# MrTornado24/FENeRF

Hardware: AMD Instinct MI355X
Metric: rays/s/GPU forward render (128x128, 24+24 samples, H=256 FiLM-SIREN + 32x96^3 grid) (higher is better)
Workload: dtype f16x3 (error-compensated fp16 MFMA, fp32 accumulate; fp32-class accuracy); 1 GPU; configs[1]: CelebA_double_semantic_texture_embedding_256_dim_96 generator, 128x128, 24+24 hierarchical samples, batch 1/GPU, forward-only render, procedural weights; img_size=128, num_steps=24, batch_per_gpu=1

## Files before the change

fenerf_amd/csrc/fenerf_siren_f16w.hip:

```cpp
#include <hip/hip_runtime.h>

#include <type_traits>

#include "fenerf_composite_ray.h"
#include "fenerf_film.h"
#include "fenerf_internal.h"
#include "fenerf_launch.h"
#include "fenerf_layout.h"
#include "fenerf_trig.h"
#include "fenerf_wave16.h"

namespace fenerf {
namespace w16 {

using namespace wave16;

typedef _Float16 half8 __attribute__((ext_vector_type(8)));
typedef _Float16 half4 __attribute__((ext_vector_type(4)));
typedef _Float16 half2 __attribute__((ext_vector_type(2)));

#define MFMA16W(a, b, c) __builtin_amdgcn_mfma_f32_16x16x32_f16((a), (b), (c), 0, 0, 0)

__device__ __forceinline__ half8 as_half8(const float4& v) { return __builtin_bit_cast(half8, v); }
template <int MODE> struct TapeW { const char* base; };
struct TapeQ { unsigned q[4]; };
__device__ __forceinline__ unsigned phase_u16(float theta) {
  const float v = __builtin_amdgcn_fractf(theta) * 65536.f;
  const unsigned c = __builtin_bit_cast(unsigned, v + 8388608.f) & 0xffffu;
  return !(__builtin_fabsf(theta) < __builtin_inff()) ? TAPE16_NONFINITE : (c == TAPE16_NONFINITE ? (v < 65535.f ? 0xfffeu : 0u) : c);
}
#ifndef FENERF_EXP_DEPHASE
#define FENERF_EXP_DEPHASE 0
#endif

struct WStream {
  bool skip;
  unsigned long long g_next;
  unsigned voff;
  unsigned ring_lds;
  const char* ring_lane;
  bool early;
};

__device__ __forceinline__ void ws_issue(WStream& w, int slot) {
  const unsigned m0 = w.ring_lds + (unsigned)slot * (CH * 1024);
  if (!w.skip) glds_1k_s(reinterpret_cast<const void*>(w.g_next), w.voff, m0);
  w.g_next += CH * 1024;
}

template <bool LO = true>
__device__ __forceinline__ AK ws_read(const WStream& w, int slot, int spl) {
  AK a;
  if (LO) ring_read_lo(a, w.ring_lane, slot, spl);
  else { a.lo[0] = make_float4(0.f, 0.f, 0.f, 0.f); a.lo[1] = a.lo[0]; }
  ring_read_hi(a, w.ring_lane, slot, spl);
  return a;
}

__device__ __forceinline__ void ws_step(WStream& w, int i, bool early) {
  const bool sync = (i & 1) == 0;
  if (sync) {
    wait_vmcnt<DPF - 3>();
    __builtin_amdgcn_s_barrier();
  }
  LDS_FENCE();
  if (early)
    ws_issue(w, (i + DPF) % NSLOT);
}
__device__ __forceinline__ void ws_issue_late(WStream& w, int i, bool early) {
  if (!early) ws_issue(w, (i + DPF) % NSLOT);
}

template <bool LO = true>
__device__ __forceinline__ void kstep_mfma(f32x4 (&acc)[2], const AK& a, const half8& bh, const half8& bl) {
  if (LO) {
    acc[0] = MFMA16W(as_half8(a.lo[0]), bh, acc[0]);
    acc[1] = MFMA16W(as_half8(a.lo[1]), bh, acc[1]);
  }
  acc[0] = MFMA16W(as_half8(a.hi[0]), bl, acc[0]);
  acc[1] = MFMA16W(as_half8(a.hi[1]), bl, acc[1]);
  acc[0] = MFMA16W(as_half8(a.hi[0]), bh, acc[0]);
  acc[1] = MFMA16W(as_half8(a.hi[1]), bh, acc[1]);
}

struct FilmQ { float2 f, p; };
template <int PF4>
__device__ __forceinline__ FilmQ epi_load(int nbp, int piece, const float* film) {
  const int rt = piece >> 1, pc = piece & 1;
  FilmQ q;
  q.f = *reinterpret_cast<const float2*>(film + 32 * nbp + 8 * rt + 2 * pc);
  q.p = *reinterpret_cast<const float2*>(film + PF4 + 32 * nbp + 8 * rt + 2 * pc);
  return q;
}
template <int KS, int SAVE>
__device__ __forceinline__ void epi_compute(const f32x4 (&acc)[2], int nbp, int piece, const FilmQ& q, half8 (&yh)[KS],
                                            half8 (&yl)[KS], TapeW<SAVE> tw, int tile_odd, TapeQ& tq) {
  const int rt = piece >> 1, pc = piece & 1;
  const float2 f = q.f, p = q.p;
  if (SAVE == 1 && pc == 0) {
    const int lo = opaque((int)(threadIdx.x & 63));
    const unsigned toff = (unsigned)(((2 * (lo >> 5)) * 64 + ((lo >> 4) & 1) * 32 + 16 * tile_odd + (lo & 15)) * 16);
    st_f4_nt(tw.base + (nbp * 4 + rt) * 1024, toff, acc[rt]);
  }
  const float th0 = __builtin_fmaf(f.x, acc[rt][2 * pc + 0], p.x), th1 = __builtin_fmaf(f.y, acc[rt][2 * pc + 1], p.y);
  if (SAVE == 2) {
    tq.q[piece] = __builtin_amdgcn_perm(phase_u16(th1), phase_u16(th0), 0x05040100u);
    if (piece == 3) {
      const int lo = opaque((int)(threadIdx.x & 63));
      const u32x4 v = {tq.q[0], tq.q[1], tq.q[2], tq.q[3]};
      st_u4_nt(tw.base + nbp * 2048, (unsigned)(1024 * tile_odd + 16 * lo), v);
    }
  }
  const float s0 = sin2pi(th0);
  const float s1 = sin2pi(th1);
  const _Float16 h0 = (_Float16)__builtin_fmaf(s0, F16_ACT_SCALE, 0.f), h1 = (_Float16)__builtin_fmaf(s1, F16_ACT_SCALE, 0.f);
  half2 hp = {h0, h1}, lp = {(_Float16)__builtin_fmaf(s0, F16_ACT_SCALE, -(float)h0), (_Float16)__builtin_fmaf(s1, F16_ACT_SCALE, -(float)h1)};
  asm volatile("" : "+v"(hp), "+v"(lp));
  const int s = 4 * rt + 2 * pc;
  yh[nbp][s] = hp[0]; yh[nbp][s + 1] = hp[1];
  yl[nbp][s] = lp[0]; yl[nbp][s + 1] = lp[1];
}
template <int KS, int PF4, int SAVE>
__device__ __forceinline__ void epi_piece(const f32x4 (&acc)[2], int nbp, int piece, const float* film, half8 (&yh)[KS],
                                          half8 (&yl)[KS], TapeW<SAVE> tw, int tile_odd, TapeQ& tq) {
  epi_compute<KS, SAVE>(acc, nbp, piece, epi_load<PF4>(nbp, piece, film), yh, yl, tw, tile_odd, tq);
}
template <int KS, int PF4, int SAVE>
__device__ __forceinline__ void epi_all(const f32x4 (&acc)[2], int nbp, const float* film, half8 (&yh)[KS], half8 (&yl)[KS],
                                        TapeW<SAVE> tw, int tile_odd) {
  TapeQ tq;
#pragma unroll
  for (int pc = 0; pc < 4; ++pc) epi_piece<KS, PF4, SAVE>(acc, nbp, pc, film, yh, yl, tw, tile_odd, tq);
}

struct APipe { AK c, n; };
struct FilmQ2 { FilmQ q[4]; };
template <bool LOR = true, bool LOM = true, int PH = -1, class BOP, class LOADQ, class PIECE>
__device__ __forceinline__ void chunk_step(f32x4 (&acc)[2], APipe& a, WStream& ws, int i, int sp0, BOP bop, LOADQ loadq, PIECE piece) {
  const bool early = PH < 0 ? ws.early : PH == 0;
  constexpr int PSPL = (PH == 1 && FENERF_EXP_DEPHASE == 1) ? 0 : 1;
  ws_step(ws, i, early);
  FilmQ2 fq;
#pragma unroll
  for (int spl = 0; spl < 2; ++spl) {
    if (spl == 1) ws_issue_late(ws, i, early);
    if (spl == 0) loadq(fq);
    const AK nn = ws_read<LOR>(ws, (i + 1) % NSLOT, spl);
    __builtin_amdgcn_sched_barrier(0);
    half8 bh, bl;
    if (bop(sp0 + spl, bh, bl)) kstep_mfma<LOR && LOM>(acc, a.c, bh, bl);
    if (spl == PSPL) piece(fq);
    a.c = a.n;
    a.n = nn;
    __builtin_amdgcn_sched_barrier(0);
  }
}
template <bool LO = true, int PH = -1>
__device__ __forceinline__ void chunk_skip(APipe& a, WStream& ws, int i) {
  const bool early = PH < 0 ? ws.early : PH == 0;
  ws_step(ws, i, early);
  ws_issue_late(ws, i, early);
  a.c = ws_read<LO>(ws, (i + 1) % NSLOT, 0);
  a.n = ws_read<LO>(ws, (i + 1) % NSLOT, 1);
  __builtin_amdgcn_sched_barrier(0);
}

template <int QB>
__device__ __forceinline__ void piece_range(int qc, int& p0, int& p1) {
  constexpr int QBE = QB < 4 ? QB : 4;
  if (qc >= QBE) { p0 = p1 = 0; return; }
  p0 = 4 * qc / QBE;
  p1 = 4 * (qc + 1) / QBE;
}

template <bool FUSED> struct FuseArgs {};
template <> struct FuseArgs<true> {
  int rays_per_group, octs_per_group;
  long long groups, total_rays;
  float* z_fine;
  float* out_fine;
  CompositeParams coarse;
  CompositeParams final_;
};
#ifndef FENERF_EXP_RAY_PHASE
#define FENERF_EXP_RAY_PHASE 2
#endif
#ifndef FENERF_EXP_FUSED_MAXM
#define FENERF_EXP_FUSED_MAXM 128
#endif
constexpr int FUSED_MAXM = FENERF_EXP_FUSED_MAXM;

template <int H, bool GRID, int SAVE, bool FUSED = false, int TERMS2 = 0>
__global__ __launch_bounds__(512, 2) void siren16w_kernel(SirenParams P, int n_geo, int n_color, int n_lab, int C, FuseArgs<FUSED> F) {
  static_assert(!(FUSED && SAVE != 0), "the fused render is the no-grad path");
  static_assert(TERMS2 == 0 || (SAVE == 0 && !FUSED), "the reduced-precision forwards are plain no-grad evaluations");
  constexpr bool LOR = TERMS2 != 1;
  constexpr bool LOC = TERMS2 == 0;
  constexpr int NB = H / 32, KS = H / 32;
  constexpr int QB = (KS + 1) / 2;
  constexpr int C0_KS = KS + (GRID ? 1 : 0) + 1;
  constexpr int C0_QB = (2 * (2 * KS + (GRID ? 2 : 0) + 1) + CH - 1) / CH;
  constexpr int SQ_CHUNKS = pad_stage(NB * QB * CH) / CH;
  constexpr int C0_CHUNKS = pad_stage(NB * C0_QB * CH) / CH;
  constexpr int HEAD_CHUNKS = pad_stage(QB * CH) / CH;
  extern __shared__ __attribute__((aligned(16))) float4 smem[];

  if (P.clk && threadIdx.x == 0) {
    P.clk[(size_t)blockIdx.x * 4 + 0] = __builtin_amdgcn_s_memtime();
    P.clk[(size_t)blockIdx.x * 4 + 1] = __builtin_amdgcn_s_memrealtime();
  }
  const int lane = threadIdx.x & 63;
  const int wave = __builtin_amdgcn_readfirstlane(threadIdx.x >> 6);
  const int n = lane & 15, g = lane >> 4;
  const int L = n_geo + n_color;
  const int stage_f4 = (16 * C + 3) / 4;
  char* lds = reinterpret_cast<char*>(smem);
  char* ring = lds;
  constexpr int FILM_F = H * 4 < 1024 ? 1024 : H * 4;
  constexpr int FILM_BYTES = 2 * FILM_F;
  char* film_base = lds + NSLOT * CH * 1024 + wave * (2 * FILM_BYTES);
  float* l0_lds = reinterpret_cast<float*>(lds + NSLOT * CH * 1024 + NWAVE * 2 * FILM_BYTES);
  float* cst = l0_lds + NB * 256;
  float* stage = cst + 80 + wave * stage_f4 * 4;
  float4* ext_wave = reinterpret_cast<float4*>(cst + 80 + NWAVE * stage_f4 * 4) + wave * 256;

  for (int i = threadIdx.x; i < NB * 256; i += 512) l0_lds[i] = P.stream[i];
  if (threadIdx.x < 32) {
    cst[threadIdx.x] = P.consts[CONST_FILM_BIAS + (size_t)2 * L * H + threadIdx.x];
    cst[32 + threadIdx.x] = P.consts[CONST_HEAD_BIAS + threadIdx.x];
  } else if (threadIdx.x < 36) {
    cst[64 + threadIdx.x - 32] = P.consts[CONST_FILM_BIAS + (size_t)2 * L * H + threadIdx.x];
    cst[68 + threadIdx.x - 32] = P.consts[CONST_RGB_BIAS + threadIdx.x - 32];
  }
  CompositeParams* ray_par = reinterpret_cast<CompositeParams*>(reinterpret_cast<float4*>(cst + 80 + NWAVE * stage_f4 * 4) + NWAVE * 256);
  if constexpr (FUSED) {
    constexpr int NW = (int)(sizeof(CompositeParams) / 4);
    static_assert(sizeof(CompositeParams) % 4 == 0 && NW <= 256, "copied one dword per thread");
    const int t = threadIdx.x & 255;
    const unsigned* src = reinterpret_cast<const unsigned*>(threadIdx.x < 256 ? &F.coarse : &F.final_);
    if (t < NW) reinterpret_cast<unsigned*>(ray_par + (threadIdx.x >> 8))[t] = src[t];
  }
  wait_vmcnt<0>();
  __syncthreads();

  WStream ws;
  {
    const int spl = wave >> 2, rt = (wave >> 1) & 1, hl = wave & 1;
    const int gi = n >> 2, r = n & 3;
    const int row = 16 * (gi >> 1) + 4 * (gi & 1) + 8 * rt + r;
    const int e_old = 2 * (2 * spl + (g >> 1)) + hl;
    ws.voff = e_old * 1024 + ((g & 1) * 32 + row) * 16;
  }
  const unsigned long long g_stream = reinterpret_cast<unsigned long long>(P.stream + P.ring_offset_floats);
  ws.g_next = g_stream;
  ws.ring_lds = __builtin_amdgcn_readfirstlane(lds_addr(ring) + wave * 1024);
  ws.ring_lane = ring + lane * 16;
  ws.early = wave < NWAVE / 2;
  ws.skip = TERMS2 == 1 && (wave & 1);

  const long long ntiles = (P.P + 15) / 16;
  const long long nocts = (ntiles + NWAVE - 1) / NWAVE;
  int opg = 1;
  long long nunits = nocts;
  if constexpr (FUSED) { opg = F.octs_per_group; nunits = F.groups; }
  const int nblk = gridDim.x;
  const int nx = nblk < 8 ? nblk : 8;
  const int xcd = blockIdx.x % nx, bi = blockIdx.x / nx;
  const int blocks_in_x = nblk / nx + (xcd < nblk % nx ? 1 : 0);
  const long long o_begin = nunits * xcd / nx, o_end = nunits * (xcd + 1) / nx;

  if (P.raw_fg && o_begin + bi < o_end) {
    const long long p_first = (o_begin + bi) * opg * (NWAVE * 16);
    long long p_last = o_end * opg * (NWAVE * 16) - 1;
    if (p_last >= P.P) p_last = P.P - 1;
    film_prep_prologue(P, p_first / P.pts_per_image, p_last / P.pts_per_image, H, n_geo, n_color);
  }

#pragma unroll
  for (int i = 0; i < DPF; ++i) ws_issue(ws, i);
  wait_vmcnt<DPF - 1>();
  __builtin_amdgcn_s_barrier();
  LDS_FENCE();
  if (wave >= NWAVE / 2) __builtin_amdgcn_s_setprio(1);
  APipe a_cur;
  a_cur.c = ws_read<LOR>(ws, 0, 0);
  a_cur.n = ws_read<LOR>(ws, 0, 1);

  for (long long unit = o_begin + bi; unit < o_end; unit += blocks_in_x) {
  const int nsub = FUSED ? 2 * opg : 1;
#pragma unroll 1
  for (int sub = 0; sub < nsub; ++sub) {
    const bool fine_pass = FUSED && sub >= opg;
    const long long oct = FUSED ? unit * opg + (fine_pass ? sub - opg : sub) : unit;
    const float* z_src = P.z;
    float* out_dst = P.out;
    if constexpr (FUSED) {
      if (fine_pass) { z_src = F.z_fine; out_dst = F.out_fine; }
    }
    ws.g_next = g_stream + (unsigned long long)DPF * (CH * 1024);
    const long long tile = oct * NWAVE + wave;
    long long pt = tile * 16 + n;
    if (pt >= P.P) pt = P.P - 1;
    const long long img = __builtin_amdgcn_readfirstlane((int)(pt / P.pts_per_image));
    float px, py, pz, dx, dy, dz;
    if (P.points) {
      px = P.points[pt * 3 + 0]; py = P.points[pt * 3 + 1]; pz = P.points[pt * 3 + 2];
      if (P.pdirs) { dx = P.pdirs[pt * 3 + 0]; dy = P.pdirs[pt * 3 + 1]; dz = P.pdirs[pt * 3 + 2]; }
      else { dx = 0.f; dy = 0.f; dz = -1.f; }
    } else {
      const long long ray = pt / P.n_per_ray;
      const float zz = z_src[pt];
      const float ox = P.origins[ray * 3 + 0], oy = P.origins[ray * 3 + 1], oz = P.origins[ray * 3 + 2];
      dx = P.dirs[ray * 3 + 0]; dy = P.dirs[ray * 3 + 1]; dz = P.dirs[ray * 3 + 2];
      px = __fadd_rn(ox, __fmul_rn(dx, zz)); py = __fadd_rn(oy, __fmul_rn(dy, zz)); pz = __fadd_rn(oz, __fmul_rn(dz, zz));
      if (P.lock_view) { dx = 0.f; dy = 0.f; dz = -1.f; }
    }
    const float qx = px * P.box_scale, qy = py * P.box_scale, qz = pz * P.box_scale;
    constexpr int TL = SAVE == 2 ? H * 64 : H * 128;
    const int tile_odd = (int)(tile & 1);
    const char* tape_tile = SAVE ? uniform_ptr(reinterpret_cast<const char*>(P.tape) + (size_t)(tile >> 1) * L * TL) : nullptr;
    auto tape_of = [&](int layer) {
      TapeW<SAVE> t{SAVE ? uniform_ptr(tape_tile + (size_t)layer * TL) : nullptr};
      if (SAVE) asm volatile("s_nop 4" ::: "memory");
      return t;
    };

    const float* fp_img = P.fp + (size_t)img * L * H;
    const float* pp_img = P.pp + (size_t)img * L * H;
    auto film_issue = [&](int layer) {
      const unsigned dst = __builtin_amdgcn_readfirstlane(lds_addr(film_base) + (layer & 1) * FILM_BYTES);
      const float* gf = fp_img + (size_t)layer * H;
      const float* gp = pp_img + (size_t)layer * H;
      const unsigned vo = (unsigned)opaque(lane) * 16;
      for (int off = 0; off < H * 4; off += 1024) {
        glds_1k_s(reinterpret_cast<const char*>(gf) + off, vo, dst + off);
        glds_1k_s(reinterpret_cast<const char*>(gp) + off, vo, dst + FILM_F + off);
      }
    };
    film_issue(0);
    if (L > 1) film_issue(1);

    float e[8];
#pragma unroll
    for (int i = 0; i < 8; ++i) e[i] = 0.f;
    if (GRID) {
      const int ch0 = 16 * (g & 1) + 8 * (g >> 1);
      const float ix = ((qx + 1.f) / 2.f) * (float)(P.gw - 1);
      const float iy = ((qy + 1.f) / 2.f) * (float)(P.gh - 1);
      const float iz = ((qz + 1.f) / 2.f) * (float)(P.gd - 1);
      const float x0 = floorf(ix), y0 = floorf(iy), z0 = floorf(iz);
#pragma unroll
      for (int c = 0; c < 8; ++c) {
        const int cz = c >> 2, cy = (c >> 1) & 1, cx = c & 1;
        const float xi = x0 + cx, yi = y0 + cy, zi = z0 + cz;
        const float wx = cx ? (ix - x0) : (x0 + 1.f - ix);
        const float wy = cy ? (iy - y0) : (y0 + 1.f - iy);
        const float wz = cz ? (iz - z0) : (z0 + 1.f - iz);
        const float wgt = wx * wy * wz;
        const bool ok = xi >= 0.f && xi <= (float)(P.gw - 1) && yi >= 0.f && yi <= (float)(P.gh - 1) && zi >= 0.f &&
                        zi <= (float)(P.gd - 1);
        if (ok) {
          const long long vox = ((long long)(int)zi * P.gh + (int)yi) * P.gw + (int)xi;
          const float4* gp = reinterpret_cast<const float4*>(P.grid + vox * 32 + ch0);
#pragma unroll
          for (int q = 0; q < 2; ++q) {
            const float4 v = gp[q];
            e[4 * q + 0] += v.x * wgt; e[4 * q + 1] += v.y * wgt; e[4 * q + 2] += v.z * wgt; e[4 * q + 3] += v.w * wgt;
          }
        }
      }
    }
    if (SAVE && GRID) {
      float4* ep = reinterpret_cast<float4*>(P.tape_e + pt * 32 + 16 * (g & 1) + 8 * (g >> 1));
      ep[0] = make_float4(e[0], e[1], e[2], e[3]);
      ep[1] = make_float4(e[4], e[5], e[6], e[7]);
    }
    {
      half8 eh, el, dh, dl;
#pragma unroll
      for (int t = 0; t < 8; ++t) {
        const float v = e[t] * F16_ACT_SCALE;
        const _Float16 hh = (_Float16)v;
        eh[t] = hh; el[t] = (_Float16)(v - (float)hh);
      }
      const float d3[3] = {dx * F16_ACT_SCALE, dy * F16_ACT_SCALE, dz * F16_ACT_SCALE};
#pragma unroll
      for (int t = 0; t < 8; ++t) { dh[t] = (_Float16)0.f; dl[t] = (_Float16)0.f; }
#pragma unroll
      for (int t = 0; t < 3; ++t) {
        const float v = g == 0 ? d3[t] : 0.f;
        const _Float16 hh = (_Float16)v;
        dh[t] = hh; dl[t] = (_Float16)(v - (float)hh);
      }
      float4* ext = ext_wave + lane;
      ext[0] = __builtin_bit_cast(float4, eh); ext[64] = __builtin_bit_cast(float4, el);
      ext[128] = __builtin_bit_cast(float4, dh); ext[192] = __builtin_bit_cast(float4, dl);
    }
    wait_vmcnt<0>();
    LDS_FENCE();

    auto film_lane = [&](int layer) -> const float* {
      const int gq = opaque(lane) >> 4;
      return reinterpret_cast<const float*>(film_base + (layer & 1) * FILM_BYTES) + 16 * (gq >> 1) + 4 * (gq & 1);
    };

    half8 xh[KS], xl[KS];
    {
      const float b = g == 0 ? qx : (g == 1 ? qy : (g == 2 ? qz : 0.f));
      const int gi = n >> 2, r = n & 3;
      const float* wl = l0_lds + ((g & 1) * 32 + 16 * (gi >> 1) + 4 * (gi & 1) + r) * 4 + (g >> 1);
      const TapeW<SAVE> tw0 = tape_of(0);
#pragma unroll
      for (int nb = 0; nb < NB; ++nb) {
        f32x4 acc[2];
#pragma unroll
        for (int rt = 0; rt < 2; ++rt) {
          const f32x4 z4 = {0.f, 0.f, 0.f, 0.f};
          acc[rt] = MFMA32W(wl[nb * 256 + 8 * rt * 4], b, z4);
        }
        epi_all<KS, FILM_F / 4, SAVE>(acc, nb, film_lane(0), xh, xl, tw0, tile_odd);
      }
    }
    auto film_layer = [&](auto ph_c, int l) {
      constexpr int PH = decltype(ph_c)::value;
      const float* ff = film_lane(l);
      const TapeW<SAVE> tw = tape_of(l);
      half8 yh[KS], yl[KS];
      if (l + 1 < L) film_issue(l + 1);
      if (SQ_CHUNKS < DPF + 2) wait_vmcnt<0>();
      if (l == n_geo) {
        const float4* ext = ext_wave + opaque(lane);
        auto bop0 = [&](int sp, half8& bh, half8& bl) -> bool {
          if (sp < KS) { bh = xh[sp]; bl = xl[sp]; return true; }
          if (GRID && sp == KS) { bh = as_half8(ext[0]); bl = as_half8(ext[64]); return true; }
          if (sp == C0_KS - 1) { bh = as_half8(ext[128]); bl = as_half8(ext[192]); return true; }
          return false;
        };
        f32x4 acc_prev[2] = {{0.f, 0.f, 0.f, 0.f}, {0.f, 0.f, 0.f, 0.f}};
        TapeQ tq;
#pragma unroll
        for (int nb = 0; nb < NB; ++nb) {
          f32x4 acc[2] = {{0.f, 0.f, 0.f, 0.f}, {0.f, 0.f, 0.f, 0.f}};
#pragma unroll
          for (int qc = 0; qc < C0_QB; ++qc) {
            chunk_step<LOR, LOC, PH>(acc, a_cur, ws, nb * C0_QB + qc, 2 * qc, bop0, [&](FilmQ2& fq) {
              if (nb > 0) {
                int p0, p1;
                piece_range<C0_QB>(qc, p0, p1);
#pragma unroll
                for (int pc = 0; pc < 4; ++pc)
                  if (pc >= p0 && pc < p1) fq.q[pc] = epi_load<FILM_F / 4>(nb - 1, pc, ff);
              }
            }, [&](const FilmQ2& fq) {
              if (nb > 0) {
                int p0, p1;
                piece_range<C0_QB>(qc, p0, p1);
#pragma unroll
                for (int pc = 0; pc < 4; ++pc)
                  if (pc >= p0 && pc < p1) epi_compute<KS, SAVE>(acc_prev, nb - 1, pc, fq.q[pc], yh, yl, tw, tile_odd, tq);
              }
            });
          }
          acc_prev[0] = acc[0]; acc_prev[1] = acc[1];
        }
#pragma unroll
        for (int i = NB * C0_QB; i < C0_CHUNKS; ++i) chunk_skip<LOR, PH>(a_cur, ws, i);
        epi_all<KS, FILM_F / 4, SAVE>(acc_prev, NB - 1, ff, yh, yl, tw, tile_odd);
        {
          f32x4 acc[2] = {{0.f, 0.f, 0.f, 0.f}, {0.f, 0.f, 0.f, 0.f}};
          auto bop = [&](int sp, half8& bh, half8& bl) -> bool {
            if (sp < KS) { bh = xh[sp]; bl = xl[sp]; return true; }
            return false;
          };
#pragma unroll
          for (int qc = 0; qc < QB; ++qc) chunk_step<LOR, true, PH>(acc, a_cur, ws, qc, 2 * qc, bop, [](FilmQ2&) {}, [](const FilmQ2&) {});
#pragma unroll
          for (int i = QB; i < HEAD_CHUNKS; ++i) chunk_skip<LOR, PH>(a_cur, ws, i);
          const int lane_o = opaque(lane);
          const int n_o = lane_o & 15, f_o = 16 * (lane_o >> 5) + 4 * ((lane_o >> 4) & 1);
#pragma unroll
          for (int rt = 0; rt < 2; ++rt) {
#pragma unroll
            for (int r = 0; r < 4; ++r) {
              const int row = f_o + 8 * rt + r;
              if (row <= n_lab) {
                const int ch = row < n_lab ? row : C - 1;
                stage[n_o * C + ch] = acc[rt][r] * cst[row] + cst[32 + row];
              }
            }
          }
        }
      } else {
        auto square_stage = [&](auto lom_c) {
        constexpr bool LOM = decltype(lom_c)::value;
        auto bop = [&](int sp, half8& bh, half8& bl) -> bool {
          if (sp < KS) { bh = xh[sp]; bl = xl[sp]; return true; }
          return false;
        };
        f32x4 acc_prev[2] = {{0.f, 0.f, 0.f, 0.f}, {0.f, 0.f, 0.f, 0.f}};
        TapeQ tq;
#pragma unroll
        for (int nb = 0; nb < NB; ++nb) {
          f32x4 acc[2] = {{0.f, 0.f, 0.f, 0.f}, {0.f, 0.f, 0.f, 0.f}};
#pragma unroll
          for (int qc = 0; qc < QB; ++qc) {
            chunk_step<LOR, LOM, PH>(acc, a_cur, ws, nb * QB + qc, 2 * qc, bop, [&](FilmQ2& fq) {
              if (nb > 0) {
                int p0, p1;
                piece_range<QB>(qc, p0, p1);
#pragma unroll
                for (int pc = 0; pc < 4; ++pc)
                  if (pc >= p0 && pc < p1) fq.q[pc] = epi_load<FILM_F / 4>(nb - 1, pc, ff);
              }
            }, [&](const FilmQ2& fq) {
              if (nb > 0) {
                int p0, p1;
                piece_range<QB>(qc, p0, p1);
#pragma unroll
                for (int pc = 0; pc < 4; ++pc)
                  if (pc >= p0 && pc < p1) epi_compute<KS, SAVE>(acc_prev, nb - 1, pc, fq.q[pc], yh, yl, tw, tile_odd, tq);
              }
            });
          }
          acc_prev[0] = acc[0]; acc_prev[1] = acc[1];
        }
#pragma unroll
        for (int i = NB * QB; i < SQ_CHUNKS; ++i) chunk_skip<LOR, PH>(a_cur, ws, i);
        epi_all<KS, FILM_F / 4, SAVE>(acc_prev, NB - 1, ff, yh, yl, tw, tile_odd);
        };
        if constexpr (TERMS2 == 2) {
          if (l < n_geo) square_stage(std::true_type{}); else square_stage(std::false_type{});
        } else {
          square_stage(std::integral_constant<bool, LOR>{});
        }
      }
#pragma unroll
      for (int k = 0; k < KS; ++k) { xh[k] = yh[k]; xl[k] = yl[k]; }
    };
#pragma unroll 1
    for (int l = 1; l < L; ++l) {
#if FENERF_WAVE_HALF_COPIES
      if (ws.early) film_layer(std::integral_constant<int, 0>{}, l); else film_layer(std::integral_constant<int, 1>{}, l);
#else
      film_layer(std::integral_constant<int, -1>{}, l);
#endif
    }
    {
      constexpr int PH = -1;
      f32x4 acc[2] = {{0.f, 0.f, 0.f, 0.f}, {0.f, 0.f, 0.f, 0.f}};
      auto bop = [&](int sp, half8& bh, half8& bl) -> bool {
        if (sp < KS) { bh = xh[sp]; bl = xl[sp]; return true; }
        return false;
      };
#pragma unroll
      for (int qc = 0; qc < QB; ++qc) chunk_step<LOR, LOC, PH>(acc, a_cur, ws, qc, 2 * qc, bop, [](FilmQ2&) {}, [](const FilmQ2&) {});
#pragma unroll
      for (int i = QB; i < HEAD_CHUNKS; ++i) chunk_skip<LOR, PH>(a_cur, ws, i);
      const int lane_o = opaque(lane);
      const int n_o = lane_o & 15;
      if ((lane_o >> 4) == 0) {
#pragma unroll
        for (int r = 0; r < 3; ++r) {
          const float v = acc[0][r] * cst[64 + r] + cst[68 + r];
          stage[n_o * C + (C - 4) + r] = 1.f / (1.f + __expf(-v));
        }
      }
    }
    __builtin_amdgcn_fence(__ATOMIC_RELEASE, "wavefront");
    __builtin_amdgcn_wave_barrier();
    __builtin_amdgcn_fence(__ATOMIC_ACQUIRE, "wavefront");
    {
      const long long base = tile * 16 * C;
      const long long limit = P.P * C;
      for (int i = opaque(lane); i < 16 * C; i += 64)
        if (base + i < limit) out_dst[base + i] = stage[i];
    }
    wait_vmcnt<0>();
    __builtin_amdgcn_wave_barrier();
    if constexpr (FUSED) {
      if (FENERF_EXP_RAY_PHASE > 0 && (sub == opg - 1 || sub == nsub - 1)) {
        __builtin_amdgcn_fence(__ATOMIC_RELEASE, "workgroup");
        __builtin_amdgcn_s_barrier();
        __builtin_amdgcn_fence(__ATOMIC_ACQUIRE, "workgroup");
        float* sc = reinterpret_cast<float*>(ext_wave);
        float* s_z = sc;
        float* s_zs = sc + FUSED_MAXM;
        int* s_ord = reinterpret_cast<int*>(sc + 2 * FUSED_MAXM + 4);
        float* s_w = sc + 3 * FUSED_MAXM + 4;
        const int lane_r = opaque(lane);
        const long long ray0 = unit * F.rays_per_group;
        for (int r = wave; r < F.rays_per_group; r += NWAVE) {
          const long long ray = ray0 + r;
          if (FENERF_EXP_RAY_PHASE > 1 && ray < F.total_rays) {
#pragma unroll 1
            for (int rep = 0; rep < (FENERF_EXP_RAY_PHASE > 2 ? 2 : 1); ++rep) {
              if (!fine_pass) composite_ray<false, FUSED_MAXM>(ray_par[0], ray, lane_r, s_z, s_zs, s_ord, s_w);
              else composite_ray<true, FUSED_MAXM>(ray_par[1], ray, lane_r, s_z, s_zs, s_ord, s_w);
              __builtin_amdgcn_wave_barrier();
            }
          }
          __builtin_amdgcn_wave_barrier();
        }
        if (!fine_pass) {
          __builtin_amdgcn_fence(__ATOMIC_RELEASE, "workgroup");
          __builtin_amdgcn_s_barrier();
          __builtin_amdgcn_fence(__ATOMIC_ACQUIRE, "workgroup");
        }
        wait_vmcnt<0>();
      }
    }
  }
  }
  wait_vmcnt<0>();
  __builtin_amdgcn_s_barrier();
  if (P.clk && threadIdx.x == 0) {
    P.clk[(size_t)blockIdx.x * 4 + 2] = __builtin_amdgcn_s_memtime();
    P.clk[(size_t)blockIdx.x * 4 + 3] = __builtin_amdgcn_s_memrealtime();
  }
}

static size_t lds_bytes_16w(const FenerfModel* m, int H) {
  const int stage_f4 = (16 * m->C + 3) / 4;
  const size_t film_f = H * 4 < 1024 ? 1024 : H * 4;
  return (size_t)NSLOT * CH * 1024 + (size_t)NWAVE * 2 * (2 * film_f) + (size_t)(H / 32) * 1024 + 80 * 4 +
         (size_t)NWAVE * stage_f4 * 16 + (size_t)NWAVE * 4096;
}

template <int H, bool GRID>
static int launch_fused_t(const FenerfModel* m, const SirenParams& p, const FuseArgs<true>& F, int blocks, void* stream) {
  const size_t lds = lds_bytes_16w(m, H) + (2 * sizeof(CompositeParams) + 255) / 256 * 256;
  auto kfn = siren16w_kernel<H, GRID, 0, true>;
  if (int rc = ensure_dynamic_lds(reinterpret_cast<const void*>(kfn), lds)) return rc;
  hipLaunchKernelGGL(kfn, dim3((unsigned)blocks), dim3(512), lds, (hipStream_t)stream, p, m->n_geo, m->n_color, m->n_lab, m->C, F);
  return check_launch("fused render launch");
}

template <int H, bool GRID, int SAVE, int TERMS2 = 0>
static int launch_t(const FenerfModel* m, const SirenParams& p, void* stream) {
  const size_t lds = lds_bytes_16w(m, H);
  auto kfn = siren16w_kernel<H, GRID, SAVE, false, TERMS2>;
  if (int rc = ensure_dynamic_lds(reinterpret_cast<const void*>(kfn), lds)) return rc;
  const unsigned blocks = persistent_blocks((p.P + 15) / 16, NWAVE, m->num_cus);
  hipLaunchKernelGGL(kfn, dim3(blocks), dim3(512), lds, (hipStream_t)stream, p, m->n_geo, m->n_color, m->n_lab, m->C, FuseArgs<false>{});
  return check_launch("siren16w launch");
}

}

static int launch_siren16w_one(const FenerfModel* m, const SirenParams& q, void* stream) {
  return dispatch_width(m->H, m->grid_ch != 0, [&](auto h, auto g) {
    constexpr int H = decltype(h)::value;
    constexpr bool GRID = decltype(g)::value;
    if (q.tape && q.tape_format == FENERF_TAPE_U16) return w16::launch_t<H, GRID, 2>(m, q, stream);
    if (q.tape) return w16::launch_t<H, GRID, 1>(m, q, stream);
    if (m->forward_mode == FENERF_FORWARD_F16X2) return w16::launch_t<H, GRID, 0, 1>(m, q, stream);
    if (m->forward_mode == FENERF_FORWARD_F16X3_COLOR_X2) return w16::launch_t<H, GRID, 0, 2>(m, q, stream);
    return w16::launch_t<H, GRID, 0>(m, q, stream);
  });
}

bool fused_render_plan(const FenerfModel* m, long long B, long long R, int N, bool balanced_only, FusedRenderPlan* plan) {
  if (m->precision != FENERF_PREC_F16X3 || N < 3 || 2 * N > w16::FUSED_MAXM) return false;
  if (m->forward_mode != FENERF_FORWARD_F16X3) return false;
  int g = N, b = 128;
  while (b) { const int t = g % b; g = b; b = t; }
  const int G = 128 / g, opg = N / g;
  if (R % G != 0) return false;
  const long long groups = B * R / G, nocts = groups * opg;
  const long long cus = launch_cus(m);
  const long long blocks_f = groups < cus ? groups : cus, blocks_p = nocts < cus ? nocts : cus;
  if (balanced_only && (groups + blocks_f - 1) / blocks_f * opg > (nocts + blocks_p - 1) / blocks_p) return false;
  plan->rays_per_group = G; plan->octs_per_group = opg; plan->groups = groups; plan->blocks = (int)blocks_f;
  return true;
}

int launch_render16w_fused(const FenerfModel* m, const SirenParams& p, const FusedRenderPlan& plan, float* z_fine, float* out_fine,
                           const CompositeParams& coarse, const CompositeParams& final_, void* stream) {
  w16::FuseArgs<true> F;
  F.rays_per_group = plan.rays_per_group; F.octs_per_group = plan.octs_per_group; F.groups = plan.groups;
  F.total_rays = coarse.BR;
  F.z_fine = z_fine; F.out_fine = out_fine; F.coarse = coarse; F.final_ = final_;
  return dispatch_width(m->H, m->grid_ch != 0, [&](auto h, auto g) {
    return w16::launch_fused_t<decltype(h)::value, decltype(g)::value>(m, p, F, plan.blocks, stream);
  });
}

int launch_siren16w(const FenerfModel* m, const SirenParams& p, void* stream) {
  if (p.P <= 0) return FENERF_OK;
  if (p.pts_per_image % 32 == 0 || p.P == p.pts_per_image) return launch_siren16w_one(m, p, stream);
  const long long nimg = p.P / p.pts_per_image;
  const int L = m->L, H = m->H;
  for (long long b = 0; b < nimg; ++b) {
    SirenParams q = p;
    q.P = p.pts_per_image;
    q.fp = p.fp + (size_t)b * L * H;
    q.pp = p.pp + (size_t)b * L * H;
    if (p.raw_fg) {
      q.raw_fg = p.raw_fg + (size_t)b * m->n_geo * H; q.raw_pg = p.raw_pg + (size_t)b * m->n_geo * H;
      q.raw_fa = p.raw_fa + (size_t)b * m->n_color * H; q.raw_pa = p.raw_pa + (size_t)b * m->n_color * H;
      q.n_images = 1;
    }
    q.out = p.out + (size_t)b * p.pts_per_image * m->C;
    if (p.points) {
      q.points = p.points + (size_t)b * p.pts_per_image * 3;
      if (p.pdirs) q.pdirs = p.pdirs + (size_t)b * p.pts_per_image * 3;
    } else {
      const long long rays = p.pts_per_image / p.n_per_ray;
      q.origins = p.origins + (size_t)b * rays * 3;
      q.dirs = p.dirs + (size_t)b * rays * 3;
      q.z = p.z + (size_t)b * p.pts_per_image;
    }
    int rc = launch_siren16w_one(m, q, stream);
    if (rc) return rc;
  }
  return FENERF_OK;
}

}
```

Before: 6.055 million rays/s.

## Carry last output block's epilogue into next layer's MFMA chunks

Defers the sine/FiLM epilogue of each layer's final output block (nb=NB-1) and interleaves it with the first MFMA chunks of the next layer, so the tail epilogue no longer sits serialized after the matmul. The next layer's first chunks only consume the earlier K-slices, which are already finalized. FiLM prefetch for layer l+1 is moved later to match, epi_all now batches its loads before a scheduling barrier, and the trailing vmcnt wait is restricted to the fused path. This adds register pressure from the carried accumulators and tape state, plus ordering complexity around the K-slice dependency.

```diff
diff --git a/fenerf_amd/csrc/fenerf_siren_f16w.hip b/fenerf_amd/csrc/fenerf_siren_f16w.hip
--- a/fenerf_amd/csrc/fenerf_siren_f16w.hip
+++ b/fenerf_amd/csrc/fenerf_siren_f16w.hip
@@ -121,16 +121,15 @@
   yl[nbp][s] = lp[0]; yl[nbp][s + 1] = lp[1];
 }
 template <int KS, int PF4, int SAVE>
-__device__ __forceinline__ void epi_piece(const f32x4 (&acc)[2], int nbp, int piece, const float* film, half8 (&yh)[KS],
-                                          half8 (&yl)[KS], TapeW<SAVE> tw, int tile_odd, TapeQ& tq) {
-  epi_compute<KS, SAVE>(acc, nbp, piece, epi_load<PF4>(nbp, piece, film), yh, yl, tw, tile_odd, tq);
-}
-template <int KS, int PF4, int SAVE>
 __device__ __forceinline__ void epi_all(const f32x4 (&acc)[2], int nbp, const float* film, half8 (&yh)[KS], half8 (&yl)[KS],
                                         TapeW<SAVE> tw, int tile_odd) {
   TapeQ tq;
-#pragma unroll
-  for (int pc = 0; pc < 4; ++pc) epi_piece<KS, PF4, SAVE>(acc, nbp, pc, film, yh, yl, tw, tile_odd, tq);
+  FilmQ q[4];
+#pragma unroll
+  for (int pc = 0; pc < 4; ++pc) q[pc] = epi_load<PF4>(nbp, pc, film);
+  __builtin_amdgcn_sched_barrier(0);
+#pragma unroll
+  for (int pc = 0; pc < 4; ++pc) epi_compute<KS, SAVE>(acc, nbp, pc, q[pc], yh, yl, tw, tile_odd, tq);
 }
 
 struct APipe { AK c, n; };
@@ -203,6 +202,7 @@
   constexpr int SQ_CHUNKS = pad_stage(NB * QB * CH) / CH;
   constexpr int C0_CHUNKS = pad_stage(NB * C0_QB * CH) / CH;
   constexpr int HEAD_CHUNKS = pad_stage(QB * CH) / CH;
+  constexpr bool CARRY = QB >= 2;
   extern __shared__ __attribute__((aligned(16))) float4 smem[];
 
   if (P.clk && threadIdx.x == 0) {
@@ -405,6 +405,25 @@
     };
 
     half8 xh[KS], xl[KS];
+    f32x4 cacc[2];
+    auto carry_load = [&](int qc, FilmQ2& fq, const float* ffc) {
+      if constexpr (CARRY) {
+        int p0, p1;
+        piece_range<QB - 1>(qc, p0, p1);
+#pragma unroll
+        for (int pc = 0; pc < 4; ++pc)
+          if (pc >= p0 && pc < p1) fq.q[pc] = epi_load<FILM_F / 4>(NB - 1, pc, ffc);
+      }
+    };
+    auto carry_piece = [&](int qc, const FilmQ2& fq, TapeW<SAVE> twc, TapeQ& tqc) {
+      if constexpr (CARRY) {
+        int p0, p1;
+        piece_range<QB - 1>(qc, p0, p1);
+#pragma unroll
+        for (int pc = 0; pc < 4; ++pc)
+          if (pc >= p0 && pc < p1) epi_compute<KS, SAVE>(cacc, NB - 1, pc, fq.q[pc], xh, xl, twc, tile_odd, tqc);
+      }
+    };
     {
       const float b = g == 0 ? qx : (g == 1 ? qy : (g == 2 ? qz : 0.f));
       const int gi = n >> 2, r = n & 3;
@@ -418,7 +437,8 @@
           const f32x4 z4 = {0.f, 0.f, 0.f, 0.f};
           acc[rt] = MFMA32W(wl[nb * 256 + 8 * rt * 4], b, z4);
         }
-        epi_all<KS, FILM_F / 4, SAVE>(acc, nb, film_lane(0), xh, xl, tw0, tile_odd);
+        if (CARRY && nb == NB - 1) { cacc[0] = acc[0]; cacc[1] = acc[1]; }
+        else epi_all<KS, FILM_F / 4, SAVE>(acc, nb, film_lane(0), xh, xl, tw0, tile_odd);
       }
     }
     auto film_layer = [&](auto ph_c, int l) {
@@ -426,7 +446,14 @@
       const float* ff = film_lane(l);
       const TapeW<SAVE> tw = tape_of(l);
       half8 yh[KS], yl[KS];
-      if (l + 1 < L) film_issue(l + 1);
+      TapeW<SAVE> twc{nullptr};
+      if constexpr (CARRY) twc = tape_of(l - 1);
+      TapeQ tqc;
+      const float* ffc = ff + ((l & 1) ? -(FILM_BYTES / 4) : FILM_BYTES / 4);
+      auto film_next = [&](int nb, int qc) {
+        if (CARRY && nb == 0 && qc == QB - 2 && l + 1 < L) film_issue(l + 1);
+      };
+      if (!CARRY && l + 1 < L) film_issue(l + 1);
       if (SQ_CHUNKS < DPF + 2) wait_vmcnt<0>();
       if (l == n_geo) {
         const float4* ext = ext_wave + opaque(lane);
@@ -450,6 +477,8 @@
 #pragma unroll
                 for (int pc = 0; pc < 4; ++pc)
                   if (pc >= p0 && pc < p1) fq.q[pc] = epi_load<FILM_F / 4>(nb - 1, pc, ff);
+              } else {
+                carry_load(qc, fq, ffc);
               }
             }, [&](const FilmQ2& fq) {
               if (nb > 0) {
@@ -458,6 +487,9 @@
 #pragma unroll
                 for (int pc = 0; pc < 4; ++pc)
                   if (pc >= p0 && pc < p1) epi_compute<KS, SAVE>(acc_prev, nb - 1, pc, fq.q[pc], yh, yl, tw, tile_odd, tq);
+              } else {
+                carry_piece(qc, fq, twc, tqc);
+                film_next(nb, qc);
               }
             });
           }
@@ -465,7 +497,8 @@
         }
 #pragma unroll
         for (int i = NB * C0_QB; i < C0_CHUNKS; ++i) chunk_skip<LOR, PH>(a_cur, ws, i);
-        epi_all<KS, FILM_F / 4, SAVE>(acc_prev, NB - 1, ff, yh, yl, tw, tile_odd);
+        if constexpr (CARRY) { cacc[0] = acc_prev[0]; cacc[1] = acc_prev[1]; }
+        else epi_all<KS, FILM_F / 4, SAVE>(acc_prev, NB - 1, ff, yh, yl, tw, tile_odd);
         {
           f32x4 acc[2] = {{0.f, 0.f, 0.f, 0.f}, {0.f, 0.f, 0.f, 0.f}};
           auto bop = [&](int sp, half8& bh, half8& bl) -> bool {
@@ -511,6 +544,8 @@
 #pragma unroll
                 for (int pc = 0; pc < 4; ++pc)
                   if (pc >= p0 && pc < p1) fq.q[pc] = epi_load<FILM_F / 4>(nb - 1, pc, ff);
+              } else {
+                carry_load(qc, fq, ffc);
               }
             }, [&](const FilmQ2& fq) {
               if (nb > 0) {
@@ -519,6 +554,9 @@
 #pragma unroll
                 for (int pc = 0; pc < 4; ++pc)
                   if (pc >= p0 && pc < p1) epi_compute<KS, SAVE>(acc_prev, nb - 1, pc, fq.q[pc], yh, yl, tw, tile_odd, tq);
+              } else {
+                carry_piece(qc, fq, twc, tqc);
+                film_next(nb, qc);
               }
             });
           }
@@ -526,7 +564,8 @@
         }
 #pragma unroll
         for (int i = NB * QB; i < SQ_CHUNKS; ++i) chunk_skip<LOR, PH>(a_cur, ws, i);
-        epi_all<KS, FILM_F / 4, SAVE>(acc_prev, NB - 1, ff, yh, yl, tw, tile_odd);
+        if constexpr (CARRY) { cacc[0] = acc_prev[0]; cacc[1] = acc_prev[1]; }
+        else epi_all<KS, FILM_F / 4, SAVE>(acc_prev, NB - 1, ff, yh, yl, tw, tile_odd);
         };
         if constexpr (TERMS2 == 2) {
           if (l < n_geo) square_stage(std::true_type{}); else square_stage(std::false_type{});
@@ -535,7 +574,7 @@
         }
       }
 #pragma unroll
-      for (int k = 0; k < KS; ++k) { xh[k] = yh[k]; xl[k] = yl[k]; }
+      for (int k = 0; k < (CARRY ? KS - 1 : KS); ++k) { xh[k] = yh[k]; xl[k] = yl[k]; }
     };
 #pragma unroll 1
     for (int l = 1; l < L; ++l) {
@@ -552,8 +591,14 @@
         if (sp < KS) { bh = xh[sp]; bl = xl[sp]; return true; }
         return false;
       };
-#pragma unroll
-      for (int qc = 0; qc < QB; ++qc) chunk_step<LOR, LOC, PH>(acc, a_cur, ws, qc, 2 * qc, bop, [](FilmQ2&) {}, [](const FilmQ2&) {});
+      TapeW<SAVE> twc{nullptr};
+      if constexpr (CARRY) twc = tape_of(L - 1);
+      TapeQ tqc;
+      const float* ffc = film_lane(L - 1);
+#pragma unroll
+      for (int qc = 0; qc < QB; ++qc)
+        chunk_step<LOR, LOC, PH>(acc, a_cur, ws, qc, 2 * qc, bop, [&](FilmQ2& fq) { carry_load(qc, fq, ffc); },
+                                 [&](const FilmQ2& fq) { carry_piece(qc, fq, twc, tqc); });
 #pragma unroll
       for (int i = QB; i < HEAD_CHUNKS; ++i) chunk_skip<LOR, PH>(a_cur, ws, i);
       const int lane_o = opaque(lane);
@@ -575,7 +620,7 @@
       for (int i = opaque(lane); i < 16 * C; i += 64)
         if (base + i < limit) out_dst[base + i] = stage[i];
     }
-    wait_vmcnt<0>();
+    if constexpr (FUSED) wait_vmcnt<0>();
     __builtin_amdgcn_wave_barrier();
     if constexpr (FUSED) {
       if (FENERF_EXP_RAY_PHASE > 0 && (sub == opg - 1 || sub == nsub - 1)) {
```

New measurement: 6.078 million rays/s (median of 6 runs). About the same (+0.4%).
